# aconz2/font-ocr

Hardware: AMD Instinct MI355X
Metric: Mpixels/s scanned (95-glyph x --x-bits=2 bank) (higher is better)
Workload: dtype i8

## Files before the change

font_ocr_amd/csrc/hip/rows.hip:

```cpp
#include "mfma_common.h"

namespace focr {

typedef unsigned int v4u __attribute__((ext_vector_type(4)));
__device__ __forceinline__ void row_prefix_block(const uint32_t *__restrict__ cnt, uint32_t n, uint32_t *__restrict__ base, uint32_t *__restrict__ zero,
                                                 uint64_t *__restrict__ total_out, uint64_t *__restrict__ max_out, uint32_t *wave_sum, uint32_t *wave_max) {
    const uint32_t lane = threadIdx.x & 63, wv = threadIdx.x >> 6;
    const uint32_t seg = ((n + 15) / 16 + 255) / 256 * 256, b = min(n, wv * seg), e = min(n, b + seg);
    const v4u *cnt4 = reinterpret_cast<const v4u *>(cnt);
    uint32_t sum = 0, mx = 0;
    for (uint32_t i0 = b + 4 * lane; i0 < e; i0 += 4 * 256) {
        v4u vv[4];
#pragma unroll
        for (int q = 0; q < 4; q++) {
            vv[q] = v4u{0, 0, 0, 0};
            if (i0 + q * 256 < e) vv[q] = cnt4[(i0 + q * 256) / 4];
        }
#pragma unroll
        for (int q = 0; q < 4; q++) {
            sum += vv[q][0] + vv[q][1] + vv[q][2] + vv[q][3];
            mx = max(max(mx, max(vv[q][0], vv[q][1])), max(vv[q][2], vv[q][3]));
        }
    }
#pragma unroll
    for (int o = 32; o > 0; o >>= 1) {
        sum += (uint32_t)__shfl_xor((int)sum, o);
        mx = max(mx, (uint32_t)__shfl_xor((int)mx, o));
    }
    if (lane == 0) {
        wave_sum[wv] = sum;
        wave_max[wv] = mx;
    }
    __syncthreads();
    uint32_t carry = 0;
    for (uint32_t q = 0; q < wv; q++) carry += wave_sum[q];
    for (uint32_t i00 = b; i00 < e; i00 += 4 * 256) {
        v4u vv[4];
#pragma unroll
        for (int q = 0; q < 4; q++) {
            const uint32_t i = i00 + q * 256 + 4 * lane;
            vv[q] = v4u{0, 0, 0, 0};
            if (i < e) vv[q] = cnt4[i / 4];
        }
#pragma unroll
        for (int q = 0; q < 4; q++) {
            const uint32_t i = i00 + q * 256 + 4 * lane;
            const v4u v = vv[q];
            const uint32_t tot4 = v[0] + v[1] + v[2] + v[3];
            uint32_t incl = tot4;
#pragma unroll
            for (int o = 1; o < 64; o <<= 1) {
                const uint32_t u = __shfl_up(incl, o);
                if ((int)lane >= o) incl += u;
            }
            if (i < e) {
                const uint32_t p0 = carry + incl - tot4;
                reinterpret_cast<v4u *>(base)[i / 4] = v4u{p0, p0 + v[0], p0 + v[0] + v[1], p0 + v[0] + v[1] + v[2]};
                if (zero) reinterpret_cast<v4u *>(zero)[i / 4] = v4u{0, 0, 0, 0};
            }
            carry += __shfl(incl, 63);
        }
    }
    __syncthreads();
    if (threadIdx.x == 0) {
        uint32_t tot = 0, m = 0;
        for (int q = 0; q < 16; q++) {
            tot += wave_sum[q];
            m = max(m, wave_max[q]);
        }
        base[n] = tot;
        if (total_out) *total_out = tot;
        if (max_out) *max_out = m;
    }
}
__global__ __launch_bounds__(1024) void row_prefix_kernel(const uint32_t *__restrict__ cnt, uint32_t n, uint32_t *__restrict__ base,
                                                          uint32_t *__restrict__ zero, uint64_t *__restrict__ total_out,
                                                          uint64_t *__restrict__ max_out) {
    __shared__ uint32_t wave_sum[16], wave_max[16];
    row_prefix_block(cnt, n, base, zero, total_out, max_out, wave_sum, wave_max);
}

struct TailWork {
    uint32_t *done;
    uint32_t n_rows;
    uint32_t *hbase;
    uint64_t *total_out, *max_out;
};
__device__ __forceinline__ bool last_workgroup(uint32_t *done) {
    __shared__ uint32_t is_last;
    __syncthreads();
    if (threadIdx.x == 0) {
        __builtin_amdgcn_fence(__ATOMIC_RELEASE, "agent");
        is_last = __hip_atomic_fetch_add(done, 1u, __ATOMIC_RELAXED, __HIP_MEMORY_SCOPE_AGENT) == gridDim.x - 1;
    }
    __syncthreads();
    if (is_last) {
        __builtin_amdgcn_fence(__ATOMIC_ACQUIRE, "agent");
        if (threadIdx.x == 0) *done = 0;
    }
    return is_last != 0;
}

constexpr uint32_t XBINS = 1024;
constexpr unsigned VERIFY_THREADS = 1024;
template <int CAP, int WAVES, bool LIST, bool PAY>
__global__ __launch_bounds__(WAVES * 64) void row_sort_kernel(uint32_t n_rows, const uint32_t *__restrict__ base, const uint32_t *__restrict__ fill,
                                                              uint64_t *__restrict__ bucket, uint32_t sub_bits, uint32_t bt, uint32_t seg_mask, uint32_t xs, uint32_t n_bins,
                                                              uint32_t *__restrict__ big, unsigned long long *__restrict__ flags_word, float *__restrict__ pay,
                                                              unsigned long long limit) {
    extern __shared__ __attribute__((aligned(16))) uint32_t sort_lds[];
    constexpr int K = CAP / 64;
    const int lane = threadIdx.x & 63, wv = threadIdx.x >> 6;
    uint32_t *cur = sort_lds + (size_t)wv * (XBINS + 1 + CAP);
    uint32_t *out = cur + XBINS + 1;
    const uint32_t wave = __builtin_amdgcn_readfirstlane(blockIdx.x * WAVES + wv), n_waves = gridDim.x * WAVES;
    const uint64_t sub_mask = (1ull << sub_bits) - 1;
    const uint32_t n_items = LIST ? min(big[0], n_rows) : n_rows;
    uint32_t it = wave, r = 0, n = 0, b = 0;
    if (it < n_items) {
        r = LIST ? big[1 + it] : it;
        n = fill[r];
        b = base[r];
    }
    while (it < n_items) {
        const uint32_t it2 = it + n_waves;
        uint32_t r2 = 0, n2 = 0, b2 = 0;
        if (it2 < n_items) {
            r2 = LIST ? big[1 + it2] : it2;
            n2 = fill[r2];
            b2 = base[r2];
        }
        if (PAY && (unsigned long long)b + n > limit) {
        } else if (n > (uint32_t)CAP) {
            if (lane == 0) {
                if (LIST || !big) {
                    atomicOr(flags_word, 2ull);
                } else {
                    big[1 + atomicAdd(big, 1u)] = r;
                }
            }
        } else if (n >= 2 && n <= 64 && !LIST) {
            uint64_t *row = bucket + b;
            const uint64_t key = row[(uint32_t)lane < n ? lane : n - 1];
            float pv = 0.f;
            if (PAY) pv = pay[b + ((uint32_t)lane < n ? lane : n - 1)];
            const uint32_t klo = (uint32_t)key, khi = (uint32_t)(key >> 32);
            uint32_t rank = 0;
            for (uint32_t j = 0; j < n; j++) {
                const uint64_t other = ((uint64_t)(uint32_t)__builtin_amdgcn_readlane((int)khi, (int)j) << 32) | (uint32_t)__builtin_amdgcn_readlane((int)klo, (int)j);
                rank += other < key;
            }
            if ((uint32_t)lane < n) {
                row[rank] = key;
                if (PAY) pay[b + rank] = pv;
            }
        } else if (n >= 2) {
            uint64_t *row = bucket + b;
            uint32_t sub[K], slot[K];
            uint64_t key[K];
            float pv[PAY ? K : 1];
#pragma unroll
            for (int k = 0; k < K; k++) {
                const uint32_t j = (uint32_t)lane + 64u * k;
                key[k] = 0;
                if (PAY) pv[k] = 0.f;
                if (64u * k < n) {
                    key[k] = row[j < n ? j : n - 1];
                    if (PAY) pv[k] = pay[b + (j < n ? j : n - 1)];
                }
            }
#pragma unroll
            for (int k = 0; k < K; k++) sub[k] = (uint32_t)(key[k] & sub_mask);
            const uint32_t hi32 = (uint32_t)(key[0] >> 32), lo32 = (uint32_t)key[0];
            const uint64_t high = (((uint64_t)(uint32_t)__builtin_amdgcn_readfirstlane(hi32) << 32) | (uint64_t)(uint32_t)__builtin_amdgcn_readfirstlane(lo32)) & ~sub_mask;
            for (uint32_t i = lane; i <= n_bins; i += 64) cur[i] = 0;
            __builtin_amdgcn_fence(__ATOMIC_ACQ_REL, "wavefront");
#pragma unroll
            for (int k = 0; k < K; k++)
                if (64u * k < n && (uint32_t)lane + 64u * k < n) slot[k] = atomicAdd(&cur[((sub[k] >> bt) & seg_mask) >> xs], 1u);
            __builtin_amdgcn_fence(__ATOMIC_ACQ_REL, "wavefront");
            uint32_t carry = 0;
            for (uint32_t i0 = 0; i0 <= n_bins; i0 += 64) {
                const uint32_t i = i0 + lane, v = i < n_bins ? cur[i] : 0;
                uint32_t incl = v;
#pragma unroll
                for (int o = 1; o < 64; o <<= 1) {
                    const uint32_t u = __shfl_up(incl, o);
                    if (lane >= o) incl += u;
                }
                if (i <= n_bins) cur[i] = carry + incl - v;
                carry += __shfl(incl, 63);
            }
            __builtin_amdgcn_fence(__ATOMIC_ACQ_REL, "wavefront");
#pragma unroll
            for (int k = 0; k < K; k++)
                if (64u * k < n && (uint32_t)lane + 64u * k < n) out[cur[((sub[k] >> bt) & seg_mask) >> xs] + slot[k]] = sub[k];
            __builtin_amdgcn_fence(__ATOMIC_ACQ_REL, "wavefront");
#pragma unroll
            for (int k = 0; k < K; k++)
                if (64u * k < n && (uint32_t)lane + 64u * k < n) {
                    const uint32_t e = sub[k], bin = ((e >> bt) & seg_mask) >> xs, lo = cur[bin], hi = cur[bin + 1];
                    uint32_t rank = 0;
                    for (uint32_t i = lo; i < hi; i++) rank += out[i] < e;
                    row[lo + rank] = high | e;
                    if (PAY) pay[b + lo + rank] = pv[k];
                }
            __builtin_amdgcn_fence(__ATOMIC_ACQ_REL, "wavefront");
        }
        it = it2, r = r2, n = n2, b = b2;
    }
}

template <int MODE>
__global__ __launch_bounds__(VERIFY_THREADS, MODE == 2 ? 8 : 1) void verify_list_kernel(
    const uint64_t *__restrict__ cand, const unsigned long long *__restrict__ n_cand_p, unsigned long long cap, const VerifyArgs va, uint32_t lds_rows, const RowHist rows,
    float *__restrict__ sims, uint32_t *__restrict__ slots, uint32_t *__restrict__ row_hits, const TailWork tw) {
    extern __shared__ __attribute__((aligned(16))) v4i verify_lds[];
    __shared__ uint32_t wave_sum[16], wave_max[16];
    constexpr bool LDS = MODE == 1;
    VerifyMeta *meta = reinterpret_cast<VerifyMeta *>(verify_lds);
    v4i *needle_lds = verify_lds + 2 * va.n_templates;
    uint32_t *needle12 = reinterpret_cast<uint32_t *>(needle_lds);
    for (uint32_t i = threadIdx.x; i < 2 * va.n_templates; i += blockDim.x) verify_lds[i] = reinterpret_cast<const v4i *>(va.vmeta)[i];
    if (MODE == 1)
        for (uint32_t i = threadIdx.x; i < lds_rows; i += blockDim.x) needle_lds[i] = va.needles16[i];
    if (MODE == 2)
        for (uint32_t i = threadIdx.x; i < lds_rows; i += blockDim.x) {
            const v4i r = va.needles16[i];
            needle12[3 * i] = (uint32_t)r[0], needle12[3 * i + 1] = (uint32_t)r[1], needle12[3 * i + 2] = (uint32_t)r[2];
        }
    __syncthreads();
    const unsigned long long n = min(*n_cand_p, cap);
    const int lane = threadIdx.x & 63;
    const unsigned long long stride = (unsigned long long)gridDim.x * blockDim.x;
    const unsigned long long first = (unsigned long long)blockIdx.x * blockDim.x + (threadIdx.x & ~63u);
    uint64_t key_next = first + lane < n ? cand[first + lane] : 0;
    for (unsigned long long i0 = first; i0 < n; i0 += stride) {
        const unsigned long long i = i0 + lane;
        const bool valid = i < n;
        const uint64_t key = key_next;
        if (i + stride < n) key_next = cand[i + stride];
        float sim = 0.f;
        const bool emit = valid && (MODE == 2 ? verify_candidate_narrow(key, va, needle12, meta, &sim) : verify_candidate_meta<LDS>(key, va, needle_lds, meta, &sim));
        const uint32_t r = emit ? row_of_key(key, rows) : 0xffffffffu;
        uint32_t slot = 0xffffffffu;
        uint64_t todo = __builtin_amdgcn_ballot_w64(emit);
        while (todo) {
            const uint32_t r0 = (uint32_t)__builtin_amdgcn_readlane((int)r, (int)__builtin_ctzll(todo));
            const uint64_t peers = __builtin_amdgcn_ballot_w64(r == r0);
            uint32_t start = 0;
            if (lane == (int)__builtin_ctzll(peers)) start = atomicAdd(row_hits + r0, (uint32_t)__builtin_popcountll(peers));
            start = (uint32_t)__builtin_amdgcn_readlane((int)start, (int)__builtin_ctzll(peers));
            if (r == r0) slot = start + __builtin_amdgcn_mbcnt_hi((uint32_t)(peers >> 32), __builtin_amdgcn_mbcnt_lo((uint32_t)peers, 0u));
            todo &= ~peers;
        }
        if (valid) {
            sims[i] = sim;
            slots[i] = slot;
        }
    }
    if (last_workgroup(tw.done)) row_prefix_block(row_hits, tw.n_rows, tw.hbase, nullptr, tw.total_out, tw.max_out, wave_sum, wave_max);
}

constexpr uint32_t MAX_VERIFY_CHUNKS = 16, CHUNK_QUEUE = 128;
struct ChunkTable {
    uint32_t n;
    uint32_t t_lo[MAX_VERIFY_CHUNKS + 1];
    uint32_t row_lo[MAX_VERIFY_CHUNKS + 1];
    uint32_t data_bytes;
};
template <int ROWB>
__global__ __launch_bounds__(VERIFY_THREADS, 4) void verify_chunks_kernel(
    const uint64_t *__restrict__ cand, const unsigned long long *__restrict__ n_cand_p, unsigned long long cap, const VerifyArgs va, const ChunkTable ct,
    const uint32_t *__restrict__ vrows_t, const VerifyMeta *__restrict__ vmeta_t, const RowHist rows, float *__restrict__ sims, uint32_t *__restrict__ slots,
    uint32_t *__restrict__ row_hits, const TailWork tw) {
    extern __shared__ __attribute__((aligned(16))) v4i verify_lds[];
    __shared__ uint32_t wave_sum[16], wave_max[16];
    constexpr uint32_t ROWDW = ROWB / 4;
    VerifyMeta *meta = reinterpret_cast<VerifyMeta *>(verify_lds);
    const int lane = threadIdx.x & 63, wv = threadIdx.x >> 6;
    uint64_t *q_base = reinterpret_cast<uint64_t *>(verify_lds + ct.data_bytes / 16);
    uint64_t *q_key = q_base + (size_t)wv * CHUNK_QUEUE;
    uint32_t *q_pos = reinterpret_cast<uint32_t *>(q_base + (size_t)(VERIFY_THREADS / 64) * CHUNK_QUEUE) + (size_t)wv * CHUNK_QUEUE;
    const unsigned long long n = min(*n_cand_p, cap);
    const unsigned long long n_waves = (unsigned long long)gridDim.x * (VERIFY_THREADS / 64);
    const unsigned long long per_wave = ((n + n_waves - 1) / n_waves + 63) / 64 * 64;
    const unsigned long long wb = min(n, ((unsigned long long)blockIdx.x * (VERIFY_THREADS / 64) + wv) * per_wave), we = min(n, wb + per_wave);
    auto step = [&](uint32_t m, const VerifyMeta *meta_c, const uint32_t *rows_c) {
        const bool valid = (uint32_t)lane < m;
        const uint64_t key = valid ? q_key[lane] : 0;
        const uint32_t pos = valid ? q_pos[lane] : 0;
        float sim = 0.f;
        bool emit = false;
        if (valid) {
            if (ROWB == 12) emit = verify_candidate_narrow(key, va, rows_c, meta_c, &sim);
            else emit = verify_candidate_meta<true>(key, va, reinterpret_cast<const v4i *>(rows_c), meta_c, &sim);
        }
        const uint32_t r = emit ? row_of_key(key, rows) : 0xffffffffu;
        uint32_t slot = 0xffffffffu;
        uint64_t todo = __builtin_amdgcn_ballot_w64(emit);
        while (todo) {
            const uint32_t r0 = (uint32_t)__builtin_amdgcn_readlane((int)r, (int)__builtin_ctzll(todo));
            const uint64_t peers = __builtin_amdgcn_ballot_w64(r == r0);
            uint32_t start = 0;
            if (lane == (int)__builtin_ctzll(peers)) start = atomicAdd(row_hits + r0, (uint32_t)__builtin_popcountll(peers));
            start = (uint32_t)__builtin_amdgcn_readlane((int)start, (int)__builtin_ctzll(peers));
            if (r == r0) slot = start + __builtin_amdgcn_mbcnt_hi((uint32_t)(peers >> 32), __builtin_amdgcn_mbcnt_lo((uint32_t)peers, 0u));
            todo &= ~peers;
        }
        if (valid && pos < n) {
            sims[pos] = sim;
            slots[pos] = slot;
        }
    };
    for (uint32_t k = 0; k < ct.n; k++) {
        const uint32_t t_lo = ct.t_lo[k], t_hi = ct.t_lo[k + 1], row_lo = ct.row_lo[k], n_rows_c = ct.row_lo[k + 1] - row_lo;
        uint32_t *rows_lds = reinterpret_cast<uint32_t *>(verify_lds + 2 * (t_hi - t_lo));
        __syncthreads();
        for (uint32_t i = threadIdx.x; i < 2 * (t_hi - t_lo); i += VERIFY_THREADS) verify_lds[i] = reinterpret_cast<const v4i *>(vmeta_t + t_lo)[i];
        for (uint32_t i = threadIdx.x; i < n_rows_c * ROWDW; i += VERIFY_THREADS) rows_lds[i] = vrows_t[(size_t)row_lo * ROWDW + i];
        __syncthreads();
        const VerifyMeta *meta_c = meta - t_lo;
        const uint32_t *rows_c = rows_lds - (size_t)row_lo * ROWDW;
        uint32_t count = 0;
        for (unsigned long long i0 = wb; i0 < we; i0 += 4 * 64) {
            uint64_t key4[4];
#pragma unroll
            for (int q = 0; q < 4; q++) {
                const unsigned long long i = i0 + 64 * q + lane;
                key4[q] = i < we ? cand[i] : ~0ull;
            }
#pragma unroll
            for (int q = 0; q < 4; q++) {
                const unsigned long long i = i0 + 64 * q + lane;
                const bool valid = i < we;
                const uint64_t key = key4[q];
                const uint32_t t = va.fmt.t(key);
                const bool in = valid && ((t >= t_lo && t < t_hi) || (k + 1 == ct.n && t >= t_hi));
                const uint64_t mask = __builtin_amdgcn_ballot_w64(in);
                if (mask) {
                    if (in) {
                        const uint32_t p = count + __builtin_amdgcn_mbcnt_hi((uint32_t)(mask >> 32), __builtin_amdgcn_mbcnt_lo((uint32_t)mask, 0u));
                        q_key[p] = key;
                        q_pos[p] = (uint32_t)i;
                    }
                    count += (uint32_t)__builtin_popcountll(mask);
                    __builtin_amdgcn_fence(__ATOMIC_ACQ_REL, "wavefront");
                    if (count >= 64) {
                        step(64, meta_c, rows_c);
                        const uint32_t rest = count - 64;
                        const uint64_t kk = (uint32_t)lane < rest ? q_key[64 + lane] : 0;
                        const uint32_t pp = (uint32_t)lane < rest ? q_pos[64 + lane] : 0;
                        __builtin_amdgcn_fence(__ATOMIC_ACQ_REL, "wavefront");
                        if ((uint32_t)lane < rest) {
                            q_key[lane] = kk;
                            q_pos[lane] = pp;
                        }
                        count = rest;
                        __builtin_amdgcn_fence(__ATOMIC_ACQ_REL, "wavefront");
                    }
                }
            }
        }
        if (count) step(count, meta_c, rows_c);
        __builtin_amdgcn_fence(__ATOMIC_ACQ_REL, "wavefront");
    }
    if (last_workgroup(tw.done)) row_prefix_block(row_hits, tw.n_rows, tw.hbase, nullptr, tw.total_out, tw.max_out, wave_sum, wave_max);
}

__global__ __launch_bounds__(256) void hit_scatter_kernel(const uint64_t *__restrict__ cand, const unsigned long long *__restrict__ n_cand_p, unsigned long long cap,
                                                          const RowHist rows, const uint32_t *__restrict__ hbase, const float *__restrict__ sims,
                                                          const uint32_t *__restrict__ slots, uint64_t *__restrict__ hkeys, float *__restrict__ hsims,
                                                          unsigned long long hit_cap) {
    const unsigned long long n = min(*n_cand_p, cap);
    const unsigned long long stride = (unsigned long long)gridDim.x * blockDim.x;
    for (unsigned long long i = (unsigned long long)blockIdx.x * blockDim.x + threadIdx.x; i < n; i += stride) {
        const uint32_t slot = slots[i];
        if (slot == 0xffffffffu) continue;
        const uint64_t key = cand[i];
        const unsigned long long pos = (unsigned long long)hbase[row_of_key(key, rows)] + slot;
        if (pos < hit_cap) {
            hkeys[pos] = key;
            hsims[pos] = sims[i];
        }
    }
}


void row_segments(const focr_ctx *c, uint32_t *seg_shift, uint32_t *n_seg) {
    uint32_t sh = c->est.seg_shift;
    if (!sh) {
        while (((size_t)1 << sh) < c->pages.r_w) sh++;
        while (sh > 5 && ((size_t)1 << sh) * c->n_templates > ((size_t)1 << 19)) sh--;
    }
    *seg_shift = sh;
    *n_seg = (uint32_t)((c->pages.r_w + ((size_t)1 << sh) - 1) >> sh);
}

static size_t row_buckets(const focr_ctx *c) {
    uint32_t sh, ns;
    row_segments(c, &sh, &ns);
    return c->sub_np * c->pages.r_h * ns;
}

bool rows_applicable(const focr_ctx *c) {
    if (c->tail_mode == 0) return false;
    for (const SizeClass &sc : c->bank.classes)
        if (sc.tall) return false;
    static_assert(sizeof(VerifyMeta) == 32, "VerifyMeta is staged in LDS as two 16-byte words per template");
    return row_buckets(c) <= ((size_t)1 << 22) && c->fmt.bp + c->fmt.by <= 32 && c->n_templates <= 4096;
}

int rows2_begin(focr_ctx *c, ClearList &clear) {
    const size_t n_rows = row_buckets(c);
    const size_t padded = (n_rows + 1 + 3) / 4 * 4 + 4;
    if (!c->scratch(c->rows_hits, padded) || !c->scratch(c->rows_hbase, padded) || !c->scratch(c->rows_big, n_rows + 1 + 2))
        return fail(c, FOCR_ERR_NOMEM, "rows: hipMalloc failed");
    uint32_t *hits = c->rows_hits, *big = c->rows_big;
    if (!clear.add(hits, padded * 4)) return fail(c, FOCR_ERR_INVALID, "rows: clear list full or region too large");
    if (!clear.add(big, 8)) return fail(c, FOCR_ERR_INVALID, "rows: clear list full or region too large");
    uint32_t seg_shift, n_seg;
    row_segments(c, &seg_shift, &n_seg);
    c->row_hist = RowHist{nullptr, (uint32_t)c->pages.r_h, c->fmt.bt + c->fmt.bx, c->fmt.by, (uint32_t)c->sub_p0, c->fmt.bt, c->fmt.bx, seg_shift, n_seg};
    return FOCR_OK;
}

uint32_t rows_capacity_for(uint64_t row_max) { return row_max <= 4096 ? 4096u : 0u; }

static unsigned tail_grid(const focr_ctx *c, unsigned blocks) {
    if (!c->dbg_grid_num || !c->dbg_grid_den) return blocks;
    return (unsigned)std::max<uint64_t>(1, (uint64_t)blocks * c->dbg_grid_num / c->dbg_grid_den);
}

static int verify_mode(const focr_ctx *c, size_t *lds, uint32_t *rows_out) {
    size_t all_rows = 0;
    uint32_t max_w = 0;
    for (const TemplateConst &tc : c->bank.h_tconst) {
        all_rows += (size_t)tc.n_h * (tc.n_w > 16 ? 2u : 1u);
        max_w = std::max<uint32_t>(max_w, tc.n_w);
    }
    const size_t meta_bytes = c->n_templates * sizeof(VerifyMeta);
    const bool narrow = max_w <= 12 && meta_bytes + all_rows * 12 <= ((size_t)80 << 10) - 256;
    const bool in_lds = meta_bytes + all_rows * 16 <= ((size_t)144 << 10);
    *lds = meta_bytes + (narrow ? all_rows * 12 : in_lds ? all_rows * 16 : 0);
    *rows_out = (uint32_t)all_rows;
    return narrow ? 2 : in_lds ? 1 : 0;
}

int rows2_verify(focr_ctx *c, double thr_d, const unsigned long long *n_cand_p, size_t ub_c) {
    const uint32_t n_rows = (uint32_t)row_buckets(c);
    if (!c->scratch(c->scan_pos, (ub_c + 1) * 4) || !c->scratch(c->scan_flags, (ub_c + 1) * 4)) return fail(c, FOCR_ERR_NOMEM, "rows: hipMalloc failed");
    float *csims = c->scan_pos.as<float>();
    uint32_t *cslots = c->scan_flags.as<uint32_t>();
    const unsigned cus = c->n_cus;
    uint32_t *hits = c->rows_hits, *hbase = c->rows_hbase;
    const TailWork tw{c->d_counter + TAIL_DONE_WORD, n_rows, hbase, c->d_res + 6, c->d_res + 5};
    const bool nobody_behind = c->tail_full_chip;
    const unsigned vcus = (c->scan_cus && c->scan_cus < cus && !nobody_behind) ? std::max(cus - c->scan_cus, cus / 16) : cus;
    if (ub_c) {
        const VerifyArgs va = verify_args(c, thr_d);
        size_t lds;
        uint32_t all_rows;
        const int mode = verify_mode(c, &lds, &all_rows);
        if (mode == 0 && c->bank.vrow_bytes) {
            const bool narrow = c->bank.vrow_bytes == 12;
            const size_t queue_bytes = (size_t)(VERIFY_THREADS / 64) * CHUNK_QUEUE * 12 + 64;
            const size_t budget = ((size_t)150 << 10) - queue_bytes;
            ChunkTable ct{};
            size_t bytes = 0;
            uint32_t t0 = 0;
            bool ok = true;
            for (uint32_t t = 0; t <= c->n_templates && ok; t++) {
                const size_t add = t < c->n_templates ? sizeof(VerifyMeta) + (size_t)(c->bank.h_vrow0_t[t + 1] - c->bank.h_vrow0_t[t]) * c->bank.vrow_bytes : 0;
                if (t == c->n_templates || bytes + add > budget) {
                    if (t == t0 || ct.n == MAX_VERIFY_CHUNKS) {
                        ok = false;
                        break;
                    }
                    ct.t_lo[ct.n] = t0;
                    ct.row_lo[ct.n] = c->bank.h_vrow0_t[t0];
                    ct.data_bytes = std::max(ct.data_bytes, (uint32_t)((bytes + 15) & ~(size_t)15));
                    ct.n++;
                    t0 = t;
                    bytes = 0;
                }
                bytes += add;
            }
            if (ok) {
                ct.t_lo[ct.n] = (uint32_t)c->n_templates;
                ct.row_lo[ct.n] = c->bank.h_vrow0_t[c->n_templates];
                const size_t lds_c = (size_t)ct.data_bytes + queue_bytes;
                const unsigned nbc = tail_grid(c, (unsigned)std::max<size_t>(1, std::min<size_t>((ub_c + VERIFY_THREADS - 1) / VERIFY_THREADS, (size_t)cus)));
                hipError_t attr = hipSuccess;
#define FOCR_VERIFY_CHUNKS(R)                                                                                                                                  \
    attr = hipFuncSetAttribute(reinterpret_cast<const void *>(verify_chunks_kernel<R>), hipFuncAttributeMaxDynamicSharedMemorySize, (int)lds_c);                \
    if (attr == hipSuccess)                                                                                                                                    \
    hipLaunchKernelGGL(verify_chunks_kernel<R>, dim3(nbc), dim3(VERIFY_THREADS), lds_c, c->stream, (const uint64_t *)c->d_cand, n_cand_p, (unsigned long long)ub_c, va, \
                       ct, c->bank.d_vrows_t.as<const uint32_t>(), c->bank.d_vmeta_t.p, c->row_hist, csims, cslots, hits, tw)
                if (narrow) {
                    FOCR_VERIFY_CHUNKS(12);
                } else {
                    FOCR_VERIFY_CHUNKS(16);
                }
#undef FOCR_VERIFY_CHUNKS
                if (attr == hipSuccess) {
                    FOCR_HIP(c, hipGetLastError());
                    goto verified;
                }
                (void)hipGetLastError();
            }
        }
        const unsigned per_cu = mode == 2 ? 2u : (mode == 0 && c->n_templates * sizeof(VerifyMeta) <= ((size_t)64 << 10) ? 2u : 1u);
        const unsigned nb = tail_grid(c, (unsigned)std::max<size_t>(1, std::min<size_t>((ub_c + VERIFY_THREADS - 1) / VERIFY_THREADS, (size_t)vcus * per_cu)));
#define FOCR_VERIFY_LIST(M)                                                                                                                                      \
    (void)hipFuncSetAttribute(reinterpret_cast<const void *>(verify_list_kernel<M>), hipFuncAttributeMaxDynamicSharedMemorySize, (int)lds);                       \
    hipLaunchKernelGGL(verify_list_kernel<M>, dim3(nb), dim3(VERIFY_THREADS), lds, c->stream, (const uint64_t *)c->d_cand, n_cand_p, (unsigned long long)ub_c, va, \
                       M == 0 ? 0u : all_rows, c->row_hist, csims, cslots, hits, tw)
        if (mode == 2) {
            FOCR_VERIFY_LIST(2);
        } else if (mode == 1) {
            FOCR_VERIFY_LIST(1);
        } else {
            FOCR_VERIFY_LIST(0);
        }
#undef FOCR_VERIFY_LIST
        FOCR_HIP(c, hipGetLastError());
    }
verified:
    FOCR_HIP(c, hipEventRecord(c->ev[3], c->stream));
    if (!ub_c) {
        hipLaunchKernelGGL(row_prefix_kernel, dim3(1), dim3(1024), 0, c->stream, (const uint32_t *)hits, n_rows, hbase, (uint32_t *)nullptr, c->d_res + 6, c->d_res + 5);
        FOCR_HIP(c, hipGetLastError());
    }
    return FOCR_OK;
}

int rows2_place(focr_ctx *c, const unsigned long long *n_cand_p, size_t ub_c, size_t ub_h, bool big_expected, bool sort) {
    const uint32_t n_rows = (uint32_t)row_buckets(c);
    int rc;
    if ((rc = reserve_hits(c, ub_h + 1))) return rc;
    const unsigned cus = c->n_cus;
    const uint32_t *hits = (const uint32_t *)c->rows_hits.p, *hbase = (const uint32_t *)c->rows_hbase.p;
    if (ub_c) {
        const unsigned nb = tail_grid(c, (unsigned)std::max<size_t>(1, std::min<size_t>((ub_c + 255) / 256, (size_t)cus * 16)));
        hipLaunchKernelGGL(hit_scatter_kernel, dim3(nb), dim3(256), 0, c->stream, (const uint64_t *)c->d_cand, n_cand_p, (unsigned long long)ub_c, c->row_hist, hbase,
                           (const float *)c->scan_pos.p, (const uint32_t *)c->scan_flags.p, c->d_hit_keys, c->d_hit_sims_alt, (unsigned long long)c->d_hit_keys.cap);
        FOCR_HIP(c, hipGetLastError());
    }
    if (!sort) return FOCR_OK;
    unsigned long long *flags_word = (unsigned long long *)(c->d_res + 4);
    const unsigned row_blocks = tail_grid(c, (unsigned)std::max<size_t>(1, std::min<size_t>(((size_t)n_rows + 3) / 4, (size_t)cus * 8)));
    const uint32_t seg_w = 1u << c->row_hist.seg_shift;
    uint32_t xs = 0;
    while ((seg_w >> xs) > XBINS) xs++;
    const uint32_t n_bins = seg_w >> xs;
    uint32_t *big = (uint32_t *)c->rows_big.p;
    auto k1 = row_sort_kernel<1024, 4, false, true>;
    auto k2 = row_sort_kernel<4096, 1, true, true>;
    const size_t lds1 = (size_t)4 * (XBINS + 1 + 1024) * 4, lds2 = (size_t)(XBINS + 1 + 4096) * 4;
    hipLaunchKernelGGL(k1, dim3(row_blocks), dim3(256), lds1, c->stream, n_rows, hbase, hits, c->d_hit_keys, c->fmt.bt + c->fmt.bx, c->fmt.bt, seg_w - 1, xs, n_bins,
                       big_expected ? big : (uint32_t *)nullptr, flags_word, c->d_hit_sims_alt, (unsigned long long)c->d_hit_keys.cap);
    FOCR_HIP(c, hipGetLastError());
    if (big_expected) {
        hipLaunchKernelGGL(k2, dim3(cus), dim3(64), lds2, c->stream, n_rows, hbase, hits, c->d_hit_keys, c->fmt.bt + c->fmt.bx, c->fmt.bt, seg_w - 1, xs, n_bins, big, flags_word,
                           c->d_hit_sims_alt, (unsigned long long)c->d_hit_keys.cap);
        FOCR_HIP(c, hipGetLastError());
    }
    return FOCR_OK;
}

}
```

Before: 33600.

## Add wave-uniform verify path with scalar row base and 32-bit offsets

After: 33810 (median of 4 runs). About the same (+0.6%).

```diff
diff --git a/font_ocr_amd/csrc/hip/rows.hip b/font_ocr_amd/csrc/hip/rows.hip
--- a/font_ocr_amd/csrc/hip/rows.hip
+++ b/font_ocr_amd/csrc/hip/rows.hip
@@ -1,4 +1,5 @@
 #include "mfma_common.h"
+#include "verify_forms.h"
 
 namespace focr {
 
@@ -232,6 +233,7 @@
     __syncthreads();
     const unsigned long long n = min(*n_cand_p, cap);
     const int lane = threadIdx.x & 63;
+    const bool off32 = pages_within_u32(va);
     const unsigned long long stride = (unsigned long long)gridDim.x * blockDim.x;
     const unsigned long long first = (unsigned long long)blockIdx.x * blockDim.x + (threadIdx.x & ~63u);
     uint64_t key_next = first + lane < n ? cand[first + lane] : 0;
@@ -241,7 +243,12 @@
         const uint64_t key = key_next;
         if (i + stride < n) key_next = cand[i + stride];
         float sim = 0.f;
-        const bool emit = valid && (MODE == 2 ? verify_candidate_narrow(key, va, needle12, meta, &sim) : verify_candidate_meta<LDS>(key, va, needle_lds, meta, &sim));
+        bool emit;
+        if (MODE != 0 && off32) {
+            emit = verify_step<MODE == 2 ? 3 : 4>(valid, key, va, needle12, meta, &sim);
+        } else {
+            emit = valid && (MODE == 2 ? verify_candidate_narrow(key, va, needle12, meta, &sim) : verify_candidate_meta<LDS>(key, va, needle_lds, meta, &sim));
+        }
         const uint32_t r = emit ? row_of_key(key, rows) : 0xffffffffu;
         uint32_t slot = 0xffffffffu;
         uint64_t todo = __builtin_amdgcn_ballot_w64(emit);
diff --git a/font_ocr_amd/csrc/hip/verify_forms.h b/font_ocr_amd/csrc/hip/verify_forms.h
--- /dev/null
+++ b/font_ocr_amd/csrc/hip/verify_forms.h
@@ -0,0 +1,210 @@
+#pragma once
+#include "mfma_common.h"
+
+namespace focr {
+
+typedef const __attribute__((address_space(1))) uint8_t *page_ptr;
+__device__ __forceinline__ page_ptr uniform_row(page_ptr p) {
+    asm volatile("" : "+s"(p));
+    return p;
+}
+
+template <int ND>
+__device__ __forceinline__ void load_dwords_b1(page_ptr p, uint32_t (&a)[4]) {
+    typedef uint32_t u32_b1 __attribute__((aligned(1)));
+    typedef uint32_t v2u __attribute__((ext_vector_type(2)));
+    typedef uint32_t v3u __attribute__((ext_vector_type(3)));
+    typedef uint32_t v4u_ __attribute__((ext_vector_type(4)));
+    typedef v2u v2u_b1 __attribute__((aligned(1)));
+    typedef v3u v3u_b1 __attribute__((aligned(1)));
+    typedef v4u_ v4u_b1 __attribute__((aligned(1)));
+    if (ND == 1) {
+        a[0] = *(const __attribute__((address_space(1))) u32_b1 *)p;
+    } else if (ND == 2) {
+        const v2u v = *(const __attribute__((address_space(1))) v2u_b1 *)p;
+        a[0] = v[0], a[1] = v[1];
+    } else if (ND == 3) {
+        const v3u v = *(const __attribute__((address_space(1))) v3u_b1 *)p;
+        a[0] = v[0], a[1] = v[1], a[2] = v[2];
+    } else {
+        const v4u_ v = *(const __attribute__((address_space(1))) v4u_b1 *)p;
+        a[0] = v[0], a[1] = v[1], a[2] = v[2], a[3] = v[3];
+    }
+}
+
+__device__ __forceinline__ uint32_t keep_mask(uint32_t w, int k) {
+    return w >= (uint32_t)(4 * k + 4) ? 0xffffffffu : (w <= (uint32_t)(4 * k) ? 0u : ((1u << (8 * (w - 4 * k))) - 1u));
+}
+
+template <int ROWDW, int FM, int ND, int J0, int N>
+__device__ __forceinline__ void rows_block(const uint32_t (*a)[4], const uint32_t *nd, const uint32_t (&keep)[4], uint32_t &acc, uint32_t &s_p, uint32_t &s2_p) {
+#pragma unroll
+    for (int jj = 0; jj < N; jj++) {
+#pragma unroll
+        for (int k = 0; k < ND; k++) {
+            const uint32_t aw = k < FM ? a[J0 + jj][k] : a[J0 + jj][k] & keep[k], b = nd[ROWDW * jj + k];
+            acc = __builtin_amdgcn_udot4(aw, b, acc, false);
+            s_p = __builtin_amdgcn_udot4(aw, 0x01010101u, s_p, false);
+            s2_p = __builtin_amdgcn_udot4(aw, aw, s2_p, false);
+        }
+    }
+}
+
+template <int ROWDW, int CH, bool BLOCKS, int FM, int ND>
+__device__ __forceinline__ void window_sums_uniform(const uint8_t *pages, uint32_t pitch, uint32_t off, const uint32_t *nd, uint32_t h, uint32_t w,
+                                                    uint32_t &acc, uint32_t &s_p, uint32_t &s2_p) {
+    static_assert(FM <= ND && ND <= ROWDW, "dwords covered by all <= dwords reached by any <= dwords of a row");
+    static_assert(!BLOCKS || CH == 8, "the last chunk's blocks are 4 + 2 + 1 rows");
+    uint32_t keep[4];
+#pragma unroll
+    for (int k = 0; k < 4; k++) keep[k] = keep_mask(w, k);
+    page_ptr rp = uniform_row((page_ptr)pages);
+    if (BLOCKS) {
+        uint32_t j0 = 0;
+        for (; j0 + CH <= h; j0 += CH) {
+            asm volatile("" : "+v"(off));
+            uint32_t a[CH][4];
+#pragma unroll
+            for (int jj = 0; jj < CH; jj++) {
+                load_dwords_b1<ND>(rp + off, a[jj]);
+                rp = uniform_row(rp + pitch);
+            }
+            rows_block<ROWDW, FM, ND, 0, CH>(a, nd + ROWDW * j0, keep, acc, s_p, s2_p);
+        }
+        const uint32_t r = h - j0;
+        if (r) {
+            asm volatile("" : "+v"(off));
+            const uint32_t r4 = r & 4, r6 = r & 6;
+            uint32_t a[CH][4];
+#pragma unroll
+            for (int s = 0; s < 7; s++) {
+                const uint32_t row = s < 4 ? (uint32_t)s : s < 6 ? r4 + (uint32_t)(s - 4) : r6;
+                load_dwords_b1<ND>(uniform_row(rp + (size_t)row * pitch) + off, a[s]);
+            }
+            const uint32_t *ndj = nd + ROWDW * j0;
+            if (r & 4) rows_block<ROWDW, FM, ND, 0, 4>(a, ndj, keep, acc, s_p, s2_p);
+            if (r & 2) rows_block<ROWDW, FM, ND, 4, 2>(a, ndj + ROWDW * r4, keep, acc, s_p, s2_p);
+            if (r & 1) rows_block<ROWDW, FM, ND, 6, 1>(a, ndj + ROWDW * r6, keep, acc, s_p, s2_p);
+        }
+    } else {
+        for (uint32_t j0 = 0; j0 < h; j0 += CH) {
+            asm volatile("" : "+v"(off));
+            uint32_t a[CH][4];
+#pragma unroll
+            for (int jj = 0; jj < CH; jj++) {
+                load_dwords_b1<ND>(rp + off, a[jj]);
+                rp = uniform_row(rp + pitch);
+            }
+#pragma unroll
+            for (int jj = 0; jj < CH; jj++)
+                if (j0 + jj < h) rows_block<ROWDW, FM, ND, 0, 1>(a + jj, nd + ROWDW * (j0 + jj), keep, acc, s_p, s2_p);
+        }
+    }
+}
+
+template <int ROWDW, int CH>
+__device__ __forceinline__ void window_sums_lane(const uint8_t *pages, uint32_t pitch, uint32_t off, const uint32_t *nd, uint32_t h, uint32_t w,
+                                                 uint32_t h_max, uint32_t halves_max, uint32_t &acc, uint32_t &s_p, uint32_t &s2_p) {
+    const uint32_t halves = ROWDW == 4 && w > 16 ? 2 : 1;
+    for (uint32_t hf = 0; hf < halves_max; hf++) {
+        const uint32_t w_here = hf < halves ? min(w - 16 * hf, 16u) : 0u;
+        const uint32_t h_here = hf < halves ? h : 0u;
+        uint32_t keep[4];
+#pragma unroll
+        for (int k = 0; k < 4; k++) keep[k] = keep_mask(w_here, k);
+        page_ptr rp = uniform_row((page_ptr)pages + 16 * hf);
+        for (uint32_t j0 = 0; j0 < h_max; j0 += CH) {
+            asm volatile("" : "+v"(off));
+            uint32_t a[CH][4];
+#pragma unroll
+            for (int jj = 0; jj < CH; jj++) {
+                load_dwords_b1<ROWDW>(rp + off, a[jj]);
+                rp = uniform_row(rp + pitch);
+            }
+#pragma unroll
+            for (int jj = 0; jj < CH; jj++) {
+                const uint32_t j = j0 + jj;
+                if (j < h_here) {
+#pragma unroll
+                    for (int k = 0; k < ROWDW; k++) {
+                        const uint32_t aw = a[jj][k] & keep[k], b = nd[ROWDW * (j * halves + hf) + k];
+                        acc = __builtin_amdgcn_udot4(aw, b, acc, false);
+                        s_p = __builtin_amdgcn_udot4(aw, 0x01010101u, s_p, false);
+                        s2_p = __builtin_amdgcn_udot4(aw, aw, s2_p, false);
+                    }
+                }
+            }
+        }
+    }
+}
+
+__device__ __forceinline__ bool pages_within_u32(const VerifyArgs &va) {
+    return (unsigned long long)va.n_pages * va.rows_alloc * va.pitch <= 0xffff0000ull;
+}
+
+template <int ROWDW>
+__device__ __forceinline__ bool verify_step(bool valid, uint64_t key, const VerifyArgs &va, const uint32_t *rows_lds, const VerifyMeta *meta, float *sim_out) {
+    constexpr int CH = ROWDW == 3 ? 8 : 16;
+    *sim_out = 0.f;
+    const uint32_t page = va.fmt.page(key), t = va.fmt.t(key), x = va.fmt.x(key), y = va.fmt.y(key);
+    const bool inside = t < va.n_templates && page < va.n_pages && x < va.r_w && y < va.r_h;
+    if (valid && !inside) atomicOr(va.flags_word, 4ull);
+    const bool ok = valid && inside;
+    const uint64_t okm = __builtin_amdgcn_ballot_w64(ok);
+    if (!okm) return false;
+    const VerifyMeta *mp = meta + (ok ? t : 0u);
+    const uint32_t w = mp->n_w, h = mp->n_h;
+    const uint32_t *nd = rows_lds + (size_t)ROWDW * (ok ? mp->row0 : 0u);
+    const uint32_t off = ok ? (page * va.rows_alloc + y) * va.pitch + x : 0u;
+    const uint32_t h0 = (uint32_t)__builtin_amdgcn_readlane((int)h, (int)__builtin_ctzll(okm));
+    const bool same_h = __builtin_amdgcn_ballot_w64(ok && h != h0) == 0;
+    const bool wide = ROWDW == 4 && __builtin_amdgcn_ballot_w64(ok && w > 16) != 0;
+    uint32_t acc = 0, s_p = 0, s2_p = 0;
+    if (same_h && !wide) {
+        uint32_t fm = 0, ndw = 0;
+#pragma unroll
+        for (int k = 0; k < ROWDW; k++) {
+            fm += __builtin_amdgcn_ballot_w64(ok && w < (uint32_t)(4 * k + 4)) == 0;
+            ndw += __builtin_amdgcn_ballot_w64(ok && w > (uint32_t)(4 * k)) != 0;
+        }
+#define FOCR_SUMS(FM, ND)                                                                              \
+    case 8 * ND + FM:                                                                                  \
+        window_sums_uniform<ROWDW, CH, CH == 8, FM, ND>(va.pages, va.pitch, off, nd, h0, w, acc, s_p, s2_p); \
+        break;
+        switch (8 * ndw + fm) {
+            FOCR_SUMS(0, 1)
+            FOCR_SUMS(1, 1)
+            FOCR_SUMS(0, 2)
+            FOCR_SUMS(1, 2)
+            FOCR_SUMS(2, 2)
+            FOCR_SUMS(0, 3)
+            FOCR_SUMS(1, 3)
+            FOCR_SUMS(2, 3)
+            FOCR_SUMS(3, 3)
+        default:
+            if constexpr (ROWDW == 4) {
+                switch (8 * ndw + fm) {
+                    FOCR_SUMS(0, 4)
+                    FOCR_SUMS(1, 4)
+                    FOCR_SUMS(2, 4)
+                    FOCR_SUMS(3, 4)
+                    FOCR_SUMS(4, 4)
+                }
+            }
+            break;
+        }
+#undef FOCR_SUMS
+    } else {
+        uint32_t h_max = h0;
+        for (uint64_t m = __builtin_amdgcn_ballot_w64(ok && h > h_max); m; m = __builtin_amdgcn_ballot_w64(ok && h > h_max))
+            h_max = (uint32_t)__builtin_amdgcn_readlane((int)h, (int)__builtin_ctzll(m));
+        window_sums_lane<ROWDW, CH>(va.pages, va.pitch, off, nd, ok ? h : 0u, w, h_max, wide ? 2u : 1u, acc, s_p, s2_p);
+    }
+    if (!ok) return false;
+    const double rnorm_p = window_rnorm(s_p, (uint64_t)s2_p, (double)(w * h));
+    const double sim = ncc_similarity(acc, s_p, mp->s_n, mp->n_recip, mp->rnorm_n, rnorm_p);
+    *sim_out = (float)sim;
+    return ncc_emits(sim, va.thr_d);
+}
+
+}
```
